# rsjahnige/CRYSTALS-Kyber

Measured on NVIDIA B200. Metric: ML-KEM-768 Encaps+Decaps ops/s, higher is better.
Workload: dtype u16/u64 integer

## Files before the change

### crystals-kyber_b200/csrc/mlkem_b200.cu

```cuda
#include "mlkem_kernels.cuh"

#include "../../include/mlkem_b200.h"

#include <algorithm>
#include <atomic>
#include <cstdio>
#include <cstdlib>
#include <cstring>
#include <mutex>
#include <vector>

namespace {

using namespace mlkem;

thread_local char tl_error[512] = "";
std::atomic<unsigned long long> g_launches{0};
int env_int(const char *name, int dflt) {
    const char *v = getenv(name);
    return v && *v ? atoi(v) : dflt;
}
constexpr int kSlots = 6;
constexpr int kDevSlots = 4;
constexpr int kHostSlots = 3;
// ... 41 lines not shown
}

#define LAUNCH(kernel, grid, block, smem, stream, ...)           \
    do {                                                         \
        auto kern_ = kernel;                                     \
        ProfEntry pe_;                                           \
        bool prof_on_;                                           \
        prof_begin(#kernel, (stream), pe_, prof_on_);            \
        kern_<<<(grid), (block), (smem), (stream)>>>(__VA_ARGS__); \
        prof_end((stream), pe_, prof_on_);                       \
        g_launches.fetch_add(1, std::memory_order_relaxed);      \
        CU(cudaGetLastError());                                  \
    } while (0)

inline unsigned cdiv(size_t a, size_t b) { return (unsigned)((a + b - 1) / b); }
inline unsigned warp_hash_grid(int n) { return cdiv((size_t)n, kWarpHashTPB / 32); }
inline unsigned warp_grid(size_t items, int warps_per_block) {
    size_t blocks = (items + warps_per_block - 1) / warps_per_block;
    const size_t cap = 148 * 16;
    return (unsigned)(blocks < cap ? blocks : cap);
}

#include "mlkem_tables.inl"

struct DeviceCtx {
    bool ready = false;
    cudaStream_t stream[kSlots] = {};
    void *ws[kSlots] = {};
    size_t ws_bytes[kSlots] = {};
    void *io[kSlots] = {};
    size_t io_bytes[kSlots] = {};
    cudaEvent_t ev_fork = nullptr, ev_join[kSlots] = {}, ev_slot[kSlots] = {};
    void *misc = nullptr;
    size_t misc_bytes = 0;
    int host_group = 0;
    std::mutex call_mutex;
    std::mutex misc_mutex;
};
DeviceCtx g_ctx[kMaxDevices];
std::mutex g_mutex;

struct DeviceGuard {
    int prev = -1;
    bool changed = false;
    int enter(int d) {
        if (cudaGetDevice(&prev) != cudaSuccess) prev = -1;
        if (prev == d) return 0;
        CU(cudaSetDevice(d));
        changed = true;
        return 0;
    }
    ~DeviceGuard() {
        if (changed && prev >= 0) cudaSetDevice(prev);
    }
};

int ensure_buffer(void **p, size_t *have, size_t need, cudaEvent_t last_use = nullptr) {
    if (*have >= need) return 0;
    if (*p) {
        if (last_use) CU(cudaEventSynchronize(last_use));
        CU(cudaMemset(*p, 0, *have));
        CU(cudaFree(*p));
    }
    *p = nullptr;
    *have = 0;
    size_t want = need + need / 8;
    CU(cudaMalloc(p, want));
    *have = want;
    return 0;
}

template <class KernelT>
int allow_smem(KernelT kernel, size_t bytes) {
    CU(cudaFuncSetAttribute(kernel, cudaFuncAttributeMaxDynamicSharedMemorySize, (int)bytes));
    CU(cudaFuncSetAttribute(kernel, cudaFuncAttributePreferredSharedMemoryCarveout, cudaSharedmemCarveoutMaxShared));
    return 0;
}
template <class P>
int allow_smem_matvec() {
    const size_t b = matvec_smem_bytes<P>();
    if (int rc = allow_smem(k_sample_matvec<P, kModeKeyGen>, b)) return rc;
    if (int rc = allow_smem(k_sample_matvec<P, kModeEncrypt>, b)) return rc;
    if (int rc = allow_smem(k_sample_matvec<P, kModeEncryptCompare>, b)) return rc;
    if (int rc = allow_smem(k_sample_matvec_list<P, kModeKeyGen>, b)) return rc;
    if (int rc = allow_smem(k_sample_matvec_list<P, kModeEncrypt>, b)) return rc;
    if (int rc = allow_smem(k_sample_matvec_list<P, kModeEncryptCompare>, b)) return rc;
    return 0;
}

int acquire(const mlkem_b200_opts *o, int *dev, DeviceCtx **ctx, DeviceGuard &guard) {
    int d = o ? o->device : -1;
    if (d < 0) CU(cudaGetDevice(&d));
    if (d >= kMaxDevices) {
        snprintf(tl_error, sizeof tl_error, "device ordinal %d out of range", d);
        return MLKEM_B200_ERR_ARG;
    }
    if (int rc = guard.enter(d)) return rc;
    std::lock_guard<std::mutex> lock(g_mutex);
    DeviceCtx &c = g_ctx[d];
    if (!c.ready) {
        cudaStream_t st[kSlots] = {};
        cudaEvent_t ev[2 * kSlots + 1] = {};
        auto create = [&]() -> int {
            TwiddleTables t;
            uint2 rc[24];
            build_tables(t, rc);
            CU(cudaMemcpyToSymbol(c_tw, &t, sizeof t));
            CU(cudaMemcpyToSymbol(g_tw, &t, sizeof t));
            CU(cudaMemcpyToSymbol(c_keccak_rc, rc, sizeof rc));
            uint32_t pow2[32];
            for (int k = 0; k < 32; k++) pow2[k] = 1u << k;
            CU(cudaMemcpyToSymbol(c_pow2, pow2, sizeof pow2));
            for (int s = 0; s < kSlots; s++) CU(cudaStreamCreateWithFlags(&st[s], cudaStreamNonBlocking));
            for (int e = 0; e < 2 * kSlots + 1; e++) CU(cudaEventCreateWithFlags(&ev[e], cudaEventDisableTiming));
            if (int r = allow_smem_matvec<P512>()) return r;
            if (int r = allow_smem_matvec<P768>()) return r;
            if (int r = allow_smem_matvec<P1024>()) return r;
            if (int r = allow_smem(k_sample_ntt_batch, 128 * kSlotWords * 4)) return r;
            return 0;
        };
        if (int r = create()) {
            for (auto s_ : st)
                if (s_) cudaStreamDestroy(s_);
            for (auto e_ : ev)
                if (e_) cudaEventDestroy(e_);
            return r;
        }
        for (int s = 0; s < kSlots; s++) {
            c.stream[s] = st[s];
            c.ev_join[s] = ev[s];
            c.ev_slot[s] = ev[kSlots + s];
        }
        c.ev_fork = ev[2 * kSlots];
        c.ready = true;
    }
    *dev = d;
    *ctx = &c;
    return 0;
}

struct Arena {
    uint8_t *base;
    size_t off = 0;
    explicit Arena(void *p) : base(static_cast<uint8_t *>(p)) {}
    template <class T>
    T *take(size_t count) {
        off = (off + 255) & ~size_t(255);
        T *p = reinterpret_cast<T *>(base + off);
        off += count * sizeof(T);
        return p;
    }
};

template <class P>
constexpr size_t ws_bytes_per_item() {
    size_t kg = 64 + 2 * P::K * 512 + 4 * P::K;
    size_t enc = P::K * 512 + (P::K + 1) * 128 + 32 + 4 * P::K;
    size_t dec = enc + 32 + 64 + 4;
    size_t m = kg > dec ? kg : dec;
    return m + 64;
}
constexpr size_t kWsSlack = 16 * 256;


template <class P, int MODE>
int launch_matvec(cudaStream_t st, Arena &ws, MatvecArgs a) {
    constexpr int K = P::K;
    const size_t rows = (size_t)a.n * K, smem = matvec_smem_bytes<P>();
    const unsigned blocks = cdiv(rows, 32), list_grid = std::min<unsigned>(blocks, 148 * 4);
#ifdef MLKEM_B200_EXPERIMENT
    static const int env_exp = env_int("MLKEM_B200_EXPERIMENT", 0);
    a.experiment = env_exp;
#endif
    if (a.group_limit >= 168 && rows > 32) {
        a.defer_list = ws.take<int>(rows);
        a.defer_count = ws.take<int>(1);
        CU(cudaMemsetAsync(a.defer_count, 0, sizeof(int), st));
        LAUNCH((k_sample_matvec<P, MODE>), blocks, 32 * K, smem, st, a);
#ifdef MLKEM_B200_EXPERIMENT
        if (env_exp & 16) return 0;
#endif
        LAUNCH((k_sample_matvec_list<P, MODE>), list_grid, 32 * K, smem, st, a);
    } else {
        a.defer_list = nullptr;
        a.defer_count = nullptr;
        LAUNCH((k_sample_matvec_list<P, MODE>), list_grid, 32 * K, smem, st, a);
    }
    return 0;
}

template <class P>
int enqueue_encrypt(cudaStream_t st, Arena &ws, int n, const uint8_t *ek, size_t ek_stride, KeySel keys, const uint8_t *m,
                    const uint8_t *seed, size_t seed_stride, uint8_t *c, const uint8_t *cmp, uint32_t *flags, int group_limit, bool fips,
                    const uint16_t *matrix = nullptr) {
    constexpr int K = P::K;
    uint16_t *yhat = ws.take<uint16_t>((size_t)n * K * 256);
    uint32_t *codes = ws.take<uint32_t>((size_t)n * (K + 1) * 32);
    if (!fips) {
        LAUNCH((k_noise<P::ETA1, true>), dim3(cdiv(n, kNoiseTPB), K), kNoiseTPB, 0, st, n, seed, seed_stride, 0, yhat, (size_t)K * 256,
               (uint32_t *)nullptr, (size_t)0, (uint8_t *)nullptr, (size_t)0, 0);
        LAUNCH((k_noise<P::ETA2, false>), dim3(cdiv(n, kNoiseTPB), K + 1), kNoiseTPB, 0, st, n, seed, seed_stride, K, (uint16_t *)nullptr,
               (size_t)0, codes, (size_t)(K + 1) * 32, (uint8_t *)nullptr, (size_t)0, 0);
    } else {
        LAUNCH((k_noise<P::ETA1, true, kRateSha3_256>), dim3(cdiv(n, kNoiseTPB), K), kNoiseTPB, 0, st, n, seed, seed_stride, 0, yhat,
               (size_t)K * 256, (uint32_t *)nullptr, (size_t)0, (uint8_t *)nullptr, (size_t)0, 0);
        LAUNCH((k_noise<P::ETA2, false, kRateSha3_256>), dim3(cdiv(n, kNoiseTPB), K + 1), kNoiseTPB, 0, st, n, seed, seed_stride, K,
               (uint16_t *)nullptr, (size_t)0, codes, (size_t)(K + 1) * 32, (uint8_t *)nullptr, (size_t)0, 0);
    }
    MatvecArgs a{};
    a.n = n;
    a.group_limit = group_limit;
    a.rho = ek + 384 * K;
    a.rho_stride = ek_stride;
    a.keys = keys;
    a.vec = yhat;
    a.vec_stride = (size_t)K * 256;
    a.addc = codes;
    a.addc_stride = (size_t)(K + 1) * 32;
    a.out = c;
    a.out_stride = P::C;
    a.cmp = cmp;
    a.flags = flags;
    EncVArgs v{};
    v.n = n;
    v.ek = ek;
    v.ek_stride = ek_stride;
    v.keys = keys;
    v.yhat = yhat;
    v.yhat_stride = (size_t)K * 256;
    v.addc = codes;
    v.addc_stride = (size_t)(K + 1) * 32;
    v.m = m;
    v.c = c;
    v.c_stride = P::C;
    v.cmp = cmp;
    v.flags = flags;
    const unsigned tgrid = warp_grid((size_t)n * K, kMatTableTPB / 32);
    if (cmp) {
        if (matrix) LAUNCH((k_matvec_table<P, kModeEncryptCompare>), tgrid, kMatTableTPB, 0, st, a, matrix);
        else if (int rc = launch_matvec<P, kModeEncryptCompare>(st, ws, a)) return rc;
        LAUNCH((k_encrypt_v<P, true>), warp_grid(n, kWarpTPB / 32), kWarpTPB, 0, st, v);
    } else {
        if (matrix) LAUNCH((k_matvec_table<P, kModeEncrypt>), tgrid, kMatTableTPB, 0, st, a, matrix);
        else if (int rc = launch_matvec<P, kModeEncrypt>(st, ws, a)) return rc;
        LAUNCH((k_encrypt_v<P, false>), warp_grid(n, kWarpTPB / 32), kWarpTPB, 0, st, v);
    }
    return 0;
}

template <class P>
int enqueue_keygen(cudaStream_t st, Arena &ws, int n, const uint8_t *d, const uint8_t *z, uint8_t *ek, uint8_t *dk, int group_limit, bool fips) {
    constexpr int K = P::K;
    const bool full = z != nullptr;
    const size_t dk_stride = full ? P::DK : P::DKPKE;
    uint8_t *rs = ws.take<uint8_t>((size_t)n * 64);
    uint16_t *se = ws.take<uint16_t>((size_t)n * 2 * K * 256);
    LAUNCH(k_keygen_G, cdiv(n, kHashTPB), kHashTPB, 0, st, n, d, (uint32_t)K, rs, ek + 384 * K, (size_t)P::EK,
           full ? dk + 768 * K : (uint8_t *)nullptr, dk_stride);
    if (!fips)
        LAUNCH((k_noise<P::ETA1, true>), dim3(cdiv(n, kNoiseTPB), 2 * K), kNoiseTPB, 0, st, n, rs + 32, (size_t)64, 0, se, (size_t)2 * K * 256,
               (uint32_t *)nullptr, (size_t)0, dk, dk_stride, K);
    else
        LAUNCH((k_noise<P::ETA1, true, kRateSha3_256>), dim3(cdiv(n, kNoiseTPB), 2 * K), kNoiseTPB, 0, st, n, rs + 32, (size_t)64, 0, se,
               (size_t)2 * K * 256, (uint32_t *)nullptr, (size_t)0, dk, dk_stride, K);
    MatvecArgs a{};
    a.n = n;
    a.group_limit = group_limit;
    a.rho = rs;
    a.rho_stride = 64;
    a.vec = se;
    a.vec_stride = (size_t)2 * K * 256;
    a.add16 = se + K * 256;
    a.add16_stride = (size_t)2 * K * 256;
    a.out = ek;
    a.out_stride = P::EK;
    a.out2 = full ? dk + 384 * K : nullptr;
    a.out2_stride = dk_stride;
    if (int rc = launch_matvec<P, kModeKeyGen>(st, ws, a)) return rc;
    if (full && n <= warp_hash_max()) LAUNCH((k_keygen_H_warp<P>), warp_hash_grid(n), kWarpHashTPB, 0, st, n, ek, z, dk);
    else if (full) LAUNCH((k_keygen_H<P>), cdiv(n, kHashTPB), kHashTPB, 0, st, n, ek, z, dk);
    return 0;
}

template <class P>
int enqueue_encaps(cudaStream_t st, Arena &ws, int n, const uint8_t *ek, const uint8_t *m, uint8_t *c, uint8_t *Kout, int group_limit, bool fips) {
    uint8_t *r = ws.take<uint8_t>((size_t)n * 32);
    if (n <= warp_hash_max()) LAUNCH((k_encaps_HG_warp<P>), warp_hash_grid(n), kWarpHashTPB, 0, st, n, ek, m, Kout, r);
    else LAUNCH((k_encaps_HG<P>), cdiv(n, kHashTPB), kHashTPB, 0, st, n, ek, m, Kout, r);
    return enqueue_encrypt<P>(st, ws, n, ek, P::EK, KeySel{}, m, r, 32, c, nullptr, nullptr, group_limit, fips);
}

template <class P>
int enqueue_encaps_keyed(cudaStream_t st, Arena &ws, int n, const uint8_t *ek, size_t ek_stride, const uint8_t *hek, KeySel keys,
                         const uint8_t *m, uint8_t *c, uint8_t *Kout, int group_limit, bool fips, const uint16_t *matrix) {
    uint8_t *r = ws.take<uint8_t>((size_t)n * 32);
    LAUNCH(k_encaps_G_keyed, cdiv(n, kHashTPB), kHashTPB, 0, st, n, hek, keys, m, Kout, r);
    return enqueue_encrypt<P>(st, ws, n, ek, ek_stride, keys, m, r, 32, c, nullptr, nullptr, group_limit, fips, matrix);
}

template <class P>
int enqueue_decaps(cudaStream_t st, Arena &ws, int n, const uint8_t *dk, KeySel keys, const uint8_t *c, uint8_t *Kout, int group_limit, bool fips,
                   const uint16_t *matrix = nullptr) {
    constexpr int K = P::K;
    uint8_t *mp = ws.take<uint8_t>((size_t)n * 32);
    uint8_t *Kr = ws.take<uint8_t>((size_t)n * 64);
    uint32_t *flags = ws.take<uint32_t>((size_t)n);
    CU(cudaMemsetAsync(flags, 0, (size_t)n * 4, st));
    LAUNCH((k_decrypt<P>), warp_grid(n, kWarpTPB / 32), kWarpTPB, 0, st, n, dk, (size_t)P::DK, keys, c, mp);
    LAUNCH((k_decaps_G<P>), cdiv(n, kHashTPB), kHashTPB, 0, st, n, mp, dk, keys, Kr);
    if (int rc = enqueue_encrypt<P>(st, ws, n, dk + 384 * K, P::DK, keys, mp, Kr + 32, 64, nullptr, c, flags, group_limit, fips, matrix)) return rc;
    if (n <= warp_hash_max()) {
        if (!fips) LAUNCH((k_decaps_J_select_warp<P>), warp_hash_grid(n), kWarpHashTPB, 0, st, n, dk, keys, c, Kr, flags, Kout);
        else LAUNCH((k_decaps_J_select_warp<P, kRateSha3_256>), warp_hash_grid(n), kWarpHashTPB, 0, st, n, dk, keys, c, Kr, flags, Kout);
        return 0;
    }
    if (!fips) LAUNCH((k_decaps_J_select<P>), cdiv(n, kHashTPB), kHashTPB, 0, st, n, dk, keys, c, Kr, flags, Kout);
    else LAUNCH((k_decaps_J_select<P, kRateSha3_256>), cdiv(n, kHashTPB), kHashTPB, 0, st, n, dk, keys, c, Kr, flags, Kout);
    return 0;
}

struct Buf {
    const void *in;
    void *out;
    size_t item_bytes;
    bool cells = false;
};

int launch_narrow(cudaStream_t st, const void *cells, void *dense, size_t bytes) {
    const size_t nw = bytes / 4;
// ... 1270 lines not shown
```

### crystals-kyber_b200/csrc/mlkem_kernels.cuh

```cuda
#pragma once
#include "mlkem_device.cuh"

namespace mlkem {

template <int K_, int ETA1_, int ETA2_, int DU_, int DV_>
struct ParamSet {
    static constexpr int K = K_, ETA1 = ETA1_, ETA2 = ETA2_, DU = DU_, DV = DV_;
    static constexpr int EK = 384 * K + 32;
    static constexpr int DKPKE = 384 * K;
    static constexpr int DK = 768 * K + 96;
    static constexpr int C1ROW = 32 * DU;
    static constexpr int C2 = 32 * DV;
    static constexpr int C = C1ROW * K + C2;
};
using P512 = ParamSet<2, 3, 2, 10, 4>;
using P768 = ParamSet<3, 2, 2, 10, 4>;
using P1024 = ParamSet<4, 2, 2, 11, 5>;

struct KeySel {
    const uint32_t *index;
    uint32_t base, nkeys;
};
__device__ __forceinline__ size_t key_row(const KeySel &k, int item) {
    if (k.index) return min(__ldg(k.index + item), k.nkeys - 1u);
// ... 329 lines not shown
#pragma unroll
    for (int m = 0; m < 4; m++) {
        uint32_t x = (t >> (6 * m)) & 7u, y = (t >> (6 * m + 3)) & 7u;
        out |= (x + 3u - y) << (4 * m);
    }
    return out;
}
__device__ __forceinline__ void cbd3_words(uint32_t w0, uint32_t w1, uint32_t w2, uint32_t &o0, uint32_t &o1) {
    uint32_t c0 = w0 & 0xFFFFFFu, c1 = (w0 >> 24) | ((w1 & 0xFFFFu) << 8), c2 = (w1 >> 16) | ((w2 & 0xFFu) << 16), c3 = w2 >> 8;
    o0 = cbd3_chunk(c0) | (cbd3_chunk(c1) << 16);
    o1 = cbd3_chunk(c2) | (cbd3_chunk(c3) << 16);
}

template <int ETA, int RATE, typename PUT>
__device__ __forceinline__ void prf_cbd_codes(const Lane seed[4], uint32_t nonce, PUT put) {
    Lane a[25];
    keccak_zero(a);
#pragma unroll
    for (int w = 0; w < 4; w++) a[w] = seed[w];
    a[4].lo = nonce | (kSfxXof << 8);
    a[RATE - 1].hi ^= 0x80000000u;
    keccak_f1600(a);
    if (ETA == 2) {
#pragma unroll
        for (int l = 0; l < 16; l++) {
            put(2 * l, cbd2_word(a[l].lo));
            put(2 * l + 1, cbd2_word(a[l].hi));
        }
    } else {
        constexpr int W1 = 2 * RATE;
        constexpr int G1 = W1 / 3;
        uint32_t o0, o1;
#pragma unroll
        for (int g = 0; g < G1; g++) {
            const int w = 3 * g;
            uint32_t w0 = (w & 1) ? a[w >> 1].hi : a[w >> 1].lo, w1 = ((w + 1) & 1) ? a[(w + 1) >> 1].hi : a[(w + 1) >> 1].lo,
                     w2 = ((w + 2) & 1) ? a[(w + 2) >> 1].hi : a[(w + 2) >> 1].lo;
            cbd3_words(w0, w1, w2, o0, o1);
            put(2 * g, o0);
            put(2 * g + 1, o1);
        }
        constexpr int LEFT = W1 - 3 * G1;
        uint32_t carry = 0;
        if (LEFT) carry = ((W1 - 1) & 1) ? a[(W1 - 1) >> 1].hi : a[(W1 - 1) >> 1].lo;
        keccak_f1600(a);
        int next = 0;
        if (LEFT) {
            cbd3_words(carry, a[0].lo, a[0].hi, o0, o1);
            put(2 * G1, o0);
            put(2 * G1 + 1, o1);
            next = 2;
        }
#pragma unroll
        for (int g = G1 + (LEFT ? 1 : 0); g < 16; g++) {
            const int w = next + 3 * (g - G1 - (LEFT ? 1 : 0));
            uint32_t w0 = (w & 1) ? a[w >> 1].hi : a[w >> 1].lo, w1 = ((w + 1) & 1) ? a[(w + 1) >> 1].hi : a[(w + 1) >> 1].lo,
                     w2 = ((w + 2) & 1) ? a[(w + 2) >> 1].hi : a[(w + 2) >> 1].lo;
            cbd3_words(w0, w1, w2, o0, o1);
            put(2 * g, o0);
            put(2 * g + 1, o1);
        }
    }
}

__device__ __forceinline__ void store_layoutC_global(const uint32_t x[8], int lane, uint16_t *dst) {
    reinterpret_cast<uint4 *>(dst)[lane] = pack_pairs(x);
}
__device__ __forceinline__ void load_layoutC_global(uint32_t x[8], int lane, const uint16_t *src) {
    unpack_pairs(__ldg(reinterpret_cast<const uint4 *>(src) + lane), x);
}

template <int ETA, bool NTT_OUT, int RATE = kRateShake128>
__global__ void __launch_bounds__(kNoiseTPB) k_noise(int n, const uint8_t *__restrict__ seeds, size_t seed_stride, int nonce0,
                                                     uint16_t *__restrict__ out16, size_t out16_stride,
                                                     uint32_t *__restrict__ outc, size_t outc_stride,
                                                     uint8_t *__restrict__ enc12, size_t enc12_stride, int enc12_polys) {
    __shared__ uint32_t s_codes[NTT_OUT ? kNoiseTPB * 33 : 1];
    __shared__ __align__(16) uint16_t s_scratch[NTT_OUT ? (kNoiseTPB / 32) * kScratchU16 : 2];
    const int p = blockIdx.y;
    const int item = blockIdx.x * kNoiseTPB + threadIdx.x;
    Lane seed[4];
#pragma unroll
    for (int w = 0; w < 4; w++) seed[w] = item < n ? load_lane(seeds + seed_stride * item + 8 * w) : Lane{0u, 0u};
    if (NTT_OUT) {
        uint32_t *mine = s_codes + 33 * threadIdx.x;
        prf_cbd_codes<ETA, RATE>(seed, (uint32_t)(nonce0 + p), [&](int w, uint32_t v) { mine[w] = v; });
        __syncwarp();
        const int lane = threadIdx.x & 31, warp = threadIdx.x >> 5;
        uint16_t *scratch = s_scratch + warp * kScratchU16;
        LaneTwiddles tw;
        load_lane_twiddles<kFmaPipe>(tw, lane);
        const uint32_t pw = nibble_weight(lane & 7);
        for (int t = 0; t < 32; t++) {
            int it = blockIdx.x * kNoiseTPB + warp * 32 + t;
            if (it >= n) break;
            const uint32_t *codes = s_codes + 33 * (warp * 32 + t) + (lane >> 3);
            uint32_t x[8];
#pragma unroll
            for (int r = 0; r < 8; r++) x[r] = nibble_fma(codes[4 * r], pw) + (kQ - 3);
            ntt_warp<kFmaPipe>(x, scratch, lane, tw);
            store_layoutC_global(x, lane, out16 + out16_stride * it + 256 * p);
            if (p < enc12_polys) {
                uint32_t *row = reinterpret_cast<uint32_t *>(enc12 + enc12_stride * it + 384 * p) + 3 * lane;
                row[0] = x[0] | (x[1] << 12) | (x[2] << 24);
                row[1] = (x[2] >> 8) | (x[3] << 4) | (x[4] << 16) | (x[5] << 28);
                row[2] = (x[5] >> 4) | (x[6] << 8) | (x[7] << 20);
            }
        }
    } else {
        if (item >= n) return;
        uint32_t buf[32];
        prf_cbd_codes<ETA, RATE>(seed, (uint32_t)(nonce0 + p), [&](int w, uint32_t v) { buf[w] = v; });
        uint4 *dst = reinterpret_cast<uint4 *>(outc + outc_stride * item + 32 * p);
#pragma unroll
        for (int v = 0; v < 8; v++) dst[v] = make_uint4(buf[4 * v], buf[4 * v + 1], buf[4 * v + 2], buf[4 * v + 3]);
    }
}

template <bool CHECKED>
__device__ __forceinline__ void parse_block(const Lane a[25], uint32_t &addr, uint32_t end_addr) {
#pragma unroll
    for (int ch = 0; ch < 7; ch++) {
        const uint32_t w[7] = {a[3 * ch].lo, a[3 * ch].hi, a[3 * ch + 1].lo, a[3 * ch + 1].hi, a[3 * ch + 2].lo, a[3 * ch + 2].hi, 0u};
#pragma unroll
        for (int m = 0; m < 16; m++) {
            const int bit = 12 * m, wi = bit >> 5, sh = bit & 31;
            uint32_t t;
            if (sh == 20) t = w[wi];
            else if (sh < 20) t = w[wi] * (1u << (20 - sh));
            else t = __funnelshift_r(w[wi], w[wi + 1], sh - 20);
            bool ok = t < (kQ << 20);
            if (CHECKED) ok = ok && (addr < end_addr);
            uint32_t d;
            asm("mul.hi.u32 %0, %1, 4096;" : "=r"(d) : "r"(t));
            if (ok) {
                asm volatile("st.shared.u16 [%0], %1;" ::"r"(addr), "h"((uint16_t)d) : "memory");
                addr += 2;
            }
        }
    }
}

__device__ __forceinline__ void mask_groups(Lane a[25], int usable) {
    const int cut = 24 * max(usable, 0);
#pragma unroll
    for (int k = 0; k < 42; k++) {
        const int lo = 32 * k;
        uint32_t m = cut <= lo ? 0xFFFFFFFFu : (cut >= lo + 32 ? 0u : (0xFFFFFFFFu << (cut - lo)));
        if (k & 1) a[k >> 1].hi |= m;
        else a[k >> 1].lo |= m;
    }
}

__device__ __forceinline__ void sample_ntt_thread(const Lane rho[4], uint32_t &b32, uint32_t &b33, uint16_t *slot, bool active,
                                                  int group_limit) {
    Lane a[25];
    const uint32_t base = (uint32_t)__cvta_generic_to_shared(slot), end_addr = base + 2 * kN;
    uint32_t addr = active ? base : end_addr;
    int groups_left = 0;
    bool need_init = true;
    while (__any_sync(kFullMask, addr < end_addr)) {
        if (need_init) {
            keccak_zero(a);
#pragma unroll
            for (int w = 0; w < 4; w++) a[w] = rho[w];
            a[4].lo = (b32 & 0xFFu) | ((b33 & 0xFFu) << 8) | (kSfxXof << 16);
            a[kRateShake128 - 1].hi ^= 0x80000000u;
            groups_left = group_limit;
            need_init = false;
        }
        keccak_f1600(a);
        const bool running = addr < end_addr;
        if (__any_sync(kFullMask, running && groups_left < 56)) {
            if (running && groups_left < 56) mask_groups(a, groups_left);
        }
        if (__all_sync(kFullMask, addr + 2 * 112 <= end_addr)) parse_block<false>(a, addr, end_addr);
        else parse_block<true>(a, addr, end_addr);
        groups_left -= 56;
        if (groups_left <= 0 && addr < end_addr) {
            b32 = (b32 + 1) & 0xFFu;
            b33 = (b33 + 1) & 0xFFu;
            addr = base;
            need_init = true;
        }
    }
}

#ifdef MLKEM_B200_EXPERIMENT
#define MLKEM_CHECK_SLOT_STORE(st, lim) \
    if ((st) + 512 < end_addr || (st) > (lim)) __trap();
#else
#define MLKEM_CHECK_SLOT_STORE(st, lim)
#endif
template <bool CHECKED>
__device__ __forceinline__ void parse_chunk3(const uint32_t w[7], uint32_t &addr, uint32_t end_addr) {
#ifndef MLKEM_B200_PARSE_ALU_ADDR
    const uint32_t one = c_pow2[0], two = c_pow2[1];
#endif
#pragma unroll
    for (int m = 0; m < 16; m++) {
        const int bit = 12 * m, wi = bit >> 5, sh = bit & 31;
        uint32_t t;
        if (sh == 20) t = w[wi];
        else if (sh < 20) t = shl_fma(w[wi], 20 - sh);
        else t = __funnelshift_r(w[wi], w[wi + 1], sh - 20);
        const bool ok = t < (kQ << 20);
        MLKEM_CHECK_SLOT_STORE(addr, CHECKED ? end_addr : end_addr - 2)
        asm volatile("st.shared.u16 [%0], %1;" ::"r"(addr), "h"((uint16_t)(t >> 20)) : "memory");
#ifndef MLKEM_B200_PARSE_ALU_ADDR
        if (CHECKED)
            asm volatile("{.reg .pred p; setp.lt.u32 p, %1, %2; setp.lt.and.u32 p, %0, %3, p; @p mad.lo.u32 %0, %4, %5, %0;}"
                         : "+r"(addr) : "r"(t), "r"(kQ << 20), "r"(end_addr), "r"(one), "r"(two));
        else
            asm volatile("{.reg .pred p; setp.lt.u32 p, %1, %2; @p mad.lo.u32 %0, %3, %4, %0;}" : "+r"(addr) : "r"(t), "r"(kQ << 20), "r"(one), "r"(two));
        (void)ok;
#else
        if (CHECKED) {
            if (ok && addr < end_addr) addr += 2;
        } else {
            if (ok) addr += 2;
        }
#endif
    }
}
template <bool CHECKED>
__device__ __forceinline__ void parse_block3(const Lane a[25], uint32_t &addr, uint32_t end_addr) {
#pragma unroll
    for (int ch = 0; ch < 7; ch++) {
        const uint32_t w[7] = {a[3 * ch].lo, a[3 * ch].hi, a[3 * ch + 1].lo, a[3 * ch + 1].hi, a[3 * ch + 2].lo, a[3 * ch + 2].hi, 0u};
        parse_chunk3<CHECKED>(w, addr, end_addr);
    }
}
__device__ __forceinline__ bool sample_ntt_three_blocks(const Lane rho[4], uint32_t b32, uint32_t b33, uint16_t *slot, int experiment = 0) {
    Lane a[25];
    const uint32_t base = (uint32_t)__cvta_generic_to_shared(slot), end_addr = base + 2 * kN;
    uint32_t addr = base;
    keccak_zero(a);
#pragma unroll
    for (int w = 0; w < 4; w++) a[w] = rho[w];
    a[4].lo = (b32 & 0xFFu) | ((b33 & 0xFFu) << 8) | (kSfxXof << 16);
    a[kRateShake128 - 1].hi ^= 0x80000000u;
#pragma unroll 1
    for (int blk = 0; blk < 3; blk++) {
        keccak_f1600(a);
#ifdef MLKEM_B200_EXPERIMENT
        if (experiment & 2) {
            addr += a[0].lo & 2;
            continue;
        }
#endif
        if (blk < 2) parse_block3<false>(a, addr, end_addr);
        else parse_block3<true>(a, addr, end_addr);
    }
    return addr >= end_addr;
}

enum MatvecMode { kModeKeyGen = 0, kModeEncrypt = 1, kModeEncryptCompare = 2 };

struct MatvecArgs {
    int n;
    int group_limit;
    const uint8_t *rho;
    size_t rho_stride;
    KeySel keys;
    const uint16_t *vec;
    size_t vec_stride;
    const uint16_t *add16;
    size_t add16_stride;
    const uint32_t *addc;
    size_t addc_stride;
    uint8_t *out;
    size_t out_stride;
    uint8_t *out2;
    size_t out2_stride;
    const uint8_t *cmp;
    uint32_t *flags;
    int *defer_list;
    int *defer_count;
#ifdef MLKEM_B200_EXPERIMENT
    int experiment;
#endif
};

constexpr int kMatvecWarpBytes = 512 + 384;
template <class P>
__host__ __device__ constexpr size_t matvec_slots_bytes() {
    return ((size_t)32 * P::K * kSlotWords * 4 + 15) & ~(size_t)15;
}
template <class P>
constexpr size_t matvec_smem_bytes() {
    return matvec_slots_bytes<P>() + (size_t)P::K * kMatvecWarpBytes + 32 * 4 + 32 * P::K;
}

struct MatvecLaneConsts {
    uint2 gam[4];
    LaneTwiddles tw;
    uint32_t pw;
};
template <int MODE>
__device__ __forceinline__ void matvec_load_consts(MatvecLaneConsts &c, int lane) {
#pragma unroll
    for (int r = 0; r < 4; r++) c.gam[r] = lane_gamma(lane + 32 * r);
    if (MODE != kModeKeyGen) load_lane_twiddles_inv<kFmaPipe>(c.tw, lane);
    c.pw = nibble_weight(lane & 7);
}
template <class P>
struct MatvecOperands {
    static constexpr int kCmpWords = (8 * P::DU + 31) / 32;
    uint32_t v[8 * P::K], cw[8], cmp[kCmpWords], ev[4];
};
template <class P, int MODE>
__device__ __forceinline__ void matvec_prefetch(MatvecOperands<P> &o, const MatvecArgs &g, int gg, int lane) {
    constexpr int K = P::K;
    if (gg < 0) return;
    const int item = gg / K, row = gg - item * K;
    const uint16_t *vec = g.vec + g.vec_stride * item;
#pragma unroll
    for (int j = 0; j < K; j++)
#pragma unroll
        for (int r = 0; r < 4; r++) {
            int t = lane + 32 * r;
            o.v[8 * j + 2 * r] = __ldg(vec + 256 * j + 2 * t);
            o.v[8 * j + 2 * r + 1] = __ldg(vec + 256 * j + 2 * t + 1);
        }
    if (MODE == kModeEncryptCompare) {
        const uint32_t *cw = reinterpret_cast<const uint32_t *>(g.cmp + g.out_stride * item + (size_t)P::C1ROW * row);
#pragma unroll
        for (int i = 0; i < MatvecOperands<P>::kCmpWords; i++) o.cmp[i] = (lane + 32 * i < 8 * P::DU) ? __ldg(cw + lane + 32 * i) : 0u;
    }
    if (MODE != kModeKeyGen) {
        const uint32_t *codes = g.addc + g.addc_stride * item + 32 * row + (lane >> 3);
#pragma unroll
        for (int r = 0; r < 8; r++) o.cw[r] = __ldg(codes + 4 * r);
    } else {
        const uint32_t *ev = reinterpret_cast<const uint32_t *>(g.add16 + g.add16_stride * item + 256 * row);
#pragma unroll
        for (int r = 0; r < 4; r++) o.ev[r] = __ldg(ev + lane + 32 * r);
    }
}

template <class P, int MODE>
__device__ __forceinline__ void matvec_row_tail(const MatvecArgs &g, int item, int row, uint32_t acc[8], const uint32_t cw8[8],
                                                const uint32_t *cmpw, const uint32_t ev4[4], uint16_t *scratch, uint8_t *stage, int lane,
                                                const LaneTwiddles &tw, uint32_t pw) {
    constexpr int kCmpWords = MatvecOperands<P>::kCmpWords;
    int nwords;
    if (MODE == kModeKeyGen) {
#pragma unroll
        for (int r = 0; r < 4; r++) {
            int t = lane + 32 * r;
            uint32_t e = ev4[r];
            uint32_t c0 = csubq(canon32(acc[2 * r]) + (e & 0xFFFFu)), c1 = csubq(canon32(acc[2 * r + 1]) + (e >> 16));
            uint32_t v = c0 | (c1 << 12);
            stage[3 * t] = (uint8_t)v;
            stage[3 * t + 1] = (uint8_t)(v >> 8);
            stage[3 * t + 2] = (uint8_t)(v >> 16);
        }
        nwords = 96;
    } else {
        uint32_t *sw = reinterpret_cast<uint32_t *>(scratch);
#pragma unroll
        for (int r = 0; r < 4; r++) {
            int t = lane + 32 * r;
            sw[sidx(2 * t) >> 1] = barrett32(acc[2 * r]) + barrett32(acc[2 * r + 1]) * 65536u;
        }
        __syncwarp();
        uint32_t x[8];
        load_scratch_C(x, scratch, lane);
        __syncwarp();
        intt_warp<kFmaPipe, false>(x, scratch, lane, tw);
#pragma unroll
        for (int r = 0; r < 8; r++) {
            uint32_t y = x[r] + nibble_fma(cw8[r], pw) + (kQ - 3);
            x[r] = compress_canon<P::DU>(canon_fma(y));
        }
        store_scratch_A(x, scratch, lane);
        __syncwarp();
        load_scratch_C(x, scratch, lane);
        pack8<P::DU>(x, stage + P::DU * lane);
        nwords = 8 * P::DU;
    }
    __syncwarp();
    const uint32_t *stw = reinterpret_cast<const uint32_t *>(stage);
    const size_t row_off = (MODE == kModeKeyGen ? 384 : P::C1ROW) * (size_t)row;
    if (MODE == kModeEncryptCompare) {
        uint32_t d = 0;
#pragma unroll
        for (int i = 0; i < kCmpWords; i++)
            if (lane + 32 * i < nwords) d |= stw[lane + 32 * i] ^ cmpw[i];
        d = __any_sync(kFullMask, d != 0) ? 1u : 0u;
        if (lane == 0) atomicOr(g.flags + item, d);
    } else {
        uint32_t *ow = reinterpret_cast<uint32_t *>(g.out + g.out_stride * item + row_off);
        for (int w = lane; w < nwords; w += 32) ow[w] = stw[w];
        if (MODE == kModeKeyGen && g.out2) {
            uint32_t *ow2 = reinterpret_cast<uint32_t *>(g.out2 + g.out2_stride * item + row_off);
            for (int w = lane; w < nwords; w += 32) ow2[w] = stw[w];
        }
    }
    __syncwarp();
}

template <class P, int MODE>
__device__ __forceinline__ void matvec_finish_rows(const MatvecArgs &g, uint32_t *s_slots, const int *s_gg, int lane, int warp,
                                                   const MatvecLaneConsts &lc, MatvecOperands<P> &nx) {
    constexpr int K = P::K;
    uint8_t *warp_area = reinterpret_cast<uint8_t *>(s_slots) + matvec_slots_bytes<P>() + warp * kMatvecWarpBytes;
    uint16_t *scratch = reinterpret_cast<uint16_t *>(warp_area);
    uint8_t *stage = warp_area + 512;
    const uint2 *gam = lc.gam;
    const LaneTwiddles &tw = lc.tw;
    const uint32_t pw = lc.pw;

    constexpr int kCmpWords = MatvecOperands<P>::kCmpWords;
#pragma unroll 1
    for (int grp = warp; grp < 32; grp += K) {
        const int gg = s_gg[grp];
        uint32_t v[8 * K], cw8[8], cmpw[kCmpWords], ev4[4];
#pragma unroll
        for (int i = 0; i < 8 * K; i++) v[i] = nx.v[i];
#pragma unroll
        for (int i = 0; i < 8; i++) cw8[i] = nx.cw[i];
#pragma unroll
        for (int i = 0; i < kCmpWords; i++) cmpw[i] = nx.cmp[i];
#pragma unroll
        for (int i = 0; i < 4; i++) ev4[i] = nx.ev[i];
        matvec_prefetch<P, MODE>(nx, g, grp + K < 32 ? s_gg[grp + K] : -1, lane);
        if (gg < 0) continue;
        const int item = gg / K, row = gg - item * K;
        const uint32_t slot0 = (uint32_t)__cvta_generic_to_shared(s_slots + kSlotWords * (grp * K));
        uint32_t acc[8];
#pragma unroll
        for (int r = 0; r < 8; r++) acc[r] = 0;
#pragma unroll
        for (int j = 0; j < K; j++) {
#pragma unroll
            for (int r = 0; r < 4; r++) {
                uint16_t a0, a1;
                const uint32_t ad = slot0 + 4 * (kSlotWords * j + lane + 32 * r);
                asm volatile("ld.shared.u16 %0, [%1];" : "=h"(a0) : "r"(ad));
                asm volatile("ld.shared.u16 %0, [%1+2];" : "=h"(a1) : "r"(ad));
                basemul_acc(acc[2 * r], acc[2 * r + 1], a0, a1, v[8 * j + 2 * r], v[8 * j + 2 * r + 1], gam[r]);
            }
        }
        matvec_row_tail<P, MODE>(g, item, row, acc, cw8, cmpw, ev4, scratch, stage, lane, tw, pw);
    }
}

template <class P>
__device__ __forceinline__ int *matvec_gg(uint32_t *s_slots) {
    return reinterpret_cast<int *>(reinterpret_cast<uint8_t *>(s_slots) + matvec_slots_bytes<P>() + P::K * kMatvecWarpBytes);
}

template <class P, int MODE>
__global__ void __launch_bounds__(32 * P::K) k_sample_matvec(MatvecArgs g) {
    constexpr int K = P::K;
    extern __shared__ __align__(16) uint32_t s_slots[];
    const int tid = threadIdx.x, lane = tid & 31, warp = tid >> 5;
    int *s_gg = matvec_gg<P>(s_slots);
    uint8_t *s_inc = reinterpret_cast<uint8_t *>(s_gg + 32);
    {
        const int grp = tid / K, col = tid - grp * K;
        const int gg = blockIdx.x * 32 + grp;
        const int item = gg / K, row = gg - item * K;
        const bool active = item < g.n;
        Lane rho[4];
#pragma unroll
        for (int w = 0; w < 4; w++) rho[w] = active ? load_lane(g.rho + g.rho_stride * key_row(g.keys, item) + 8 * w) : Lane{0u, 0u};
        const uint32_t b32 = MODE == kModeKeyGen ? col : row, b33 = MODE == kModeKeyGen ? row : col;
#ifdef MLKEM_B200_EXPERIMENT
        const bool complete = (g.experiment & 8) ? true
                                                 : sample_ntt_three_blocks(rho, b32, b33, reinterpret_cast<uint16_t *>(s_slots + kSlotWords * tid), g.experiment);
#else
        const bool complete = sample_ntt_three_blocks(rho, b32, b33, reinterpret_cast<uint16_t *>(s_slots + kSlotWords * tid));
#endif
        s_inc[tid] = active && !complete;
    }
    MatvecLaneConsts lc;
    matvec_load_consts<MODE>(lc, lane);
    MatvecOperands<P> nx;
    {
        const int gg = blockIdx.x * 32 + warp;
        matvec_prefetch<P, MODE>(nx, g, gg / K < g.n ? gg : -1, lane);
    }
    __syncthreads();
    {
        const int grp = warp + K * lane;
        if (grp < 32) {
            const int gg = blockIdx.x * 32 + grp;
            bool deferred = false;
#pragma unroll
            for (int j = 0; j < K; j++) deferred |= s_inc[grp * K + j] != 0;
            const bool active = gg / K < g.n;
            s_gg[grp] = (active && !deferred) ? gg : -1;
            if (active && deferred) g.defer_list[atomicAdd(g.defer_count, 1)] = gg;
        }
        __syncwarp();
    }
#ifdef MLKEM_B200_EXPERIMENT
    if (g.experiment & 1) return;
    if (g.experiment & 4) {
        matvec_finish_rows<P, MODE>(g, s_slots, s_gg, lane, warp, lc, nx);
        matvec_prefetch<P, MODE>(nx, g, s_gg[warp], lane);
    }
#endif
    matvec_finish_rows<P, MODE>(g, s_slots, s_gg, lane, warp, lc, nx);
}

template <class P, int MODE>
__global__ void __launch_bounds__(32 * P::K) k_sample_matvec_list(MatvecArgs g) {
    constexpr int K = P::K;
    extern __shared__ __align__(16) uint32_t s_slots[];
    const int tid = threadIdx.x, lane = tid & 31, warp = tid >> 5;
    int *s_gg = matvec_gg<P>(s_slots);
    MatvecLaneConsts lc;
    matvec_load_consts<MODE>(lc, lane);
    const int count = g.defer_list ? *g.defer_count : g.n * K;
    for (int base = blockIdx.x * 32; base < count; base += gridDim.x * 32) {
        {
            const int grp = tid / K, col = tid - grp * K;
            const int e = base + grp;
            const int gg = e < count ? (g.defer_list ? g.defer_list[e] : e) : -1;
            const bool active = gg >= 0;
            const int item = active ? gg / K : 0, row = gg - item * K;
            if (col == 0) s_gg[grp] = gg;
            Lane rho[4];
#pragma unroll
            for (int w = 0; w < 4; w++) rho[w] = active ? load_lane(g.rho + g.rho_stride * key_row(g.keys, item) + 8 * w) : Lane{0u, 0u};
            uint32_t b32 = MODE == kModeKeyGen ? col : row, b33 = MODE == kModeKeyGen ? row : col;
            sample_ntt_thread(rho, b32, b33, reinterpret_cast<uint16_t *>(s_slots + kSlotWords * tid), active, g.group_limit);
        }
        __syncthreads();
        MatvecOperands<P> nx;
        matvec_prefetch<P, MODE>(nx, g, s_gg[warp], lane);
        matvec_finish_rows<P, MODE>(g, s_slots, s_gg, lane, warp, lc, nx);
        __syncthreads();
    }
}


template <class P>
__global__ void __launch_bounds__(256) k_matrix_seeds(int n, const uint8_t *__restrict__ ek, size_t ek_stride, uint8_t *__restrict__ seeds) {
    constexpr int K = P::K;
    const int e = blockIdx.x * blockDim.x + threadIdx.x;
    if (e >= n * K * K) return;
    const int key = e / (K * K), rc = e - key * K * K, row = rc / K, col = rc - row * K;
    const uint8_t *rho = ek + ek_stride * key + 384 * K;
    uint8_t *out = seeds + 34 * (size_t)e;
    for (int b = 0; b < 32; b++) out[b] = rho[b];
    out[32] = (uint8_t)row;
    out[33] = (uint8_t)col;
}

__global__ void __launch_bounds__(256) k_scatter_rows(int n, int row_words, const uint8_t *__restrict__ src, size_t src_stride, KeySel slots,
                                                      uint8_t *__restrict__ dst, size_t dst_stride) {
    const size_t total = (size_t)n * row_words;
    for (size_t t = (size_t)blockIdx.x * blockDim.x + threadIdx.x; t < total; t += (size_t)gridDim.x * blockDim.x) {
        const int i = (int)(t / row_words), w = (int)(t - (size_t)i * row_words);
        const uint4 v = reinterpret_cast<const uint4 *>(src + src_stride * i)[w];
        reinterpret_cast<uint4 *>(dst + dst_stride * key_row(slots, i))[w] = v;
    }
}

__global__ void __launch_bounds__(kHashTPB) k_expand_seed(int n, const uint8_t *__restrict__ seed, unsigned long long first, uint32_t tag,
                                                          uint8_t *__restrict__ out0, uint8_t *__restrict__ out1) {
    const int j = blockIdx.x * blockDim.x + threadIdx.x;
    if (j >= n) return;
    const unsigned long long idx = first + (unsigned long long)j;
    Lane a[25];
    sponge_absorb_words<kRateSha3_256>(a, 6, kSfxXof, [&](int w) {
        if (w < 4) return load_lane(seed + 8 * w);
        return w == 4 ? Lane{(uint32_t)idx, (uint32_t)(idx >> 32)} : Lane{tag, 0u};
    });
#pragma unroll
    for (int w = 0; w < 4; w++) store_lane(out0 + 32 * (size_t)j + 8 * w, a[w]);
    if (out1) {
#pragma unroll
        for (int w = 0; w < 4; w++) store_lane(out1 + 32 * (size_t)j + 8 * w, a[4 + w]);
    }
}

#ifndef MLKEM_B200_MATTABLE_PREFETCH
#define MLKEM_B200_MATTABLE_PREFETCH 1
#endif
#ifndef MLKEM_B200_MATTABLE_BLOCKS
#define MLKEM_B200_MATTABLE_BLOCKS 1
#endif
template <class P, int MODE>
__global__ void __launch_bounds__(kMatTableTPB, MLKEM_B200_MATTABLE_BLOCKS) k_matvec_table(MatvecArgs g, const uint16_t *__restrict__ table) {
    static_assert(MODE != kModeKeyGen, "the table is kept in Encrypt order");
    constexpr int K = P::K, NW = kMatTableTPB / 32;
    __shared__ __align__(16) uint8_t s_warp[NW * kMatvecWarpBytes];
    const int lane = threadIdx.x & 31, warp = threadIdx.x >> 5;
    uint16_t *scratch = reinterpret_cast<uint16_t *>(s_warp + warp * kMatvecWarpBytes);
    uint8_t *stage = s_warp + warp * kMatvecWarpBytes + 512;
    MatvecLaneConsts lc;
    matvec_load_consts<MODE>(lc, lane);
    const int rows = g.n * K, stride = gridDim.x * NW;
    int gg = blockIdx.x * NW + warp;
    MatvecOperands<P> nx;
    if (MLKEM_B200_MATTABLE_PREFETCH) matvec_prefetch<P, MODE>(nx, g, gg < rows ? gg : -1, lane);
    constexpr int kCmpWords = MatvecOperands<P>::kCmpWords;
#pragma unroll 1
    for (; gg < rows; gg += stride) {
        if (!MLKEM_B200_MATTABLE_PREFETCH) matvec_prefetch<P, MODE>(nx, g, gg, lane);
        const int item = gg / K, row = gg - item * K;
        const uint32_t *arow = reinterpret_cast<const uint32_t *>(table + ((size_t)key_row(g.keys, item) * K + row) * K * 256);
        uint32_t aw[4 * K];
#pragma unroll
        for (int j = 0; j < K; j++)
#pragma unroll
            for (int r = 0; r < 4; r++) aw[4 * j + r] = __ldg(arow + 128 * j + lane + 32 * r);
        uint32_t v[8 * K], cw8[8], cmpw[kCmpWords], ev4[4];
#pragma unroll
        for (int i = 0; i < 8 * K; i++) v[i] = nx.v[i];
#pragma unroll
        for (int i = 0; i < 8; i++) cw8[i] = nx.cw[i];
#pragma unroll
        for (int i = 0; i < kCmpWords; i++) cmpw[i] = nx.cmp[i];
#pragma unroll
        for (int i = 0; i < 4; i++) ev4[i] = 0;
        if (MLKEM_B200_MATTABLE_PREFETCH) matvec_prefetch<P, MODE>(nx, g, gg + stride < rows ? gg + stride : -1, lane);
        uint32_t acc[8];
#pragma unroll
        for (int r = 0; r < 8; r++) acc[r] = 0;
#pragma unroll
        for (int j = 0; j < K; j++)
#pragma unroll
            for (int r = 0; r < 4; r++)
                basemul_acc(acc[2 * r], acc[2 * r + 1], aw[4 * j + r] & 0xFFFFu, aw[4 * j + r] >> 16, v[8 * j + 2 * r], v[8 * j + 2 * r + 1], lc.gam[r]);
        matvec_row_tail<P, MODE>(g, item, row, acc, cw8, cmpw, ev4, scratch, stage, lane, lc.tw, lc.pw);
    }
}

constexpr int kWarpTPB = 128;
#ifndef MLKEM_B200_PRIM_PIPE
#define MLKEM_B200_PRIM_PIPE false
#endif
constexpr bool kPrimPipe = MLKEM_B200_PRIM_PIPE;

struct EncVArgs {
    int n;
    const uint8_t *ek;
    size_t ek_stride;
    KeySel keys;
    const uint16_t *yhat;
    size_t yhat_stride;
    const uint32_t *addc;
    size_t addc_stride;
    const uint8_t *m;
    uint8_t *c;
    size_t c_stride;
    const uint8_t *cmp;
    uint32_t *flags;
};

__device__ __forceinline__ uint32_t smem_u32(const void *p) { return (uint32_t)__cvta_generic_to_shared(p); }
__device__ __forceinline__ void mbar_init(uint64_t *bar, int count) {
    asm volatile("mbarrier.init.shared::cta.b64 [%0], %1;" ::"r"(smem_u32(bar)), "r"(count) : "memory");
}
__device__ __forceinline__ void mbar_fence_init() { asm volatile("fence.mbarrier_init.release.cluster;" ::: "memory"); }
__device__ __forceinline__ void mbar_expect_tx(uint64_t *bar, uint32_t bytes) {
    asm volatile("mbarrier.arrive.expect_tx.shared::cta.b64 _, [%0], %1;" ::"r"(smem_u32(bar)), "r"(bytes) : "memory");
}
__device__ __forceinline__ void mbar_wait(uint64_t *bar, uint32_t parity) {
    asm volatile(
        "{\n"
        ".reg .pred p;\n"
        "WAIT_%=:\n"
        "mbarrier.try_wait.parity.shared::cta.b64 p, [%0], %1;\n"
        "@p bra DONE_%=;\n"
        "bra WAIT_%=;\n"
        "DONE_%=:\n"
        "}\n" ::"r"(smem_u32(bar)),
        "r"(parity)
        : "memory");
}
__device__ __forceinline__ void bulk_g2s(void *smem_dst, const void *gmem_src, uint32_t bytes, uint64_t *bar) {
    asm volatile("cp.async.bulk.shared::cluster.global.mbarrier::complete_tx::bytes [%0], [%1], %2, [%3];" ::"r"(smem_u32(smem_dst)),
                 "l"(gmem_src), "r"(bytes), "r"(smem_u32(bar))
                 : "memory");
}

// ... 448 lines not shown
```

Measured before the change: 33.73 million.

## Resume deferred matrix sampling from saved Keccak state instead of restarting

```diff
diff --git a/crystals-kyber_b200/csrc/mlkem_b200.cu b/crystals-kyber_b200/csrc/mlkem_b200.cu
--- a/crystals-kyber_b200/csrc/mlkem_b200.cu
+++ b/crystals-kyber_b200/csrc/mlkem_b200.cu
@@ -217,10 +217,12 @@
     }
 };
 
+constexpr size_t kResumeRowsPer = 16;
 template <class P>
 constexpr size_t ws_bytes_per_item() {
-    size_t kg = 64 + 2 * P::K * 512 + 4 * P::K;
-    size_t enc = P::K * 512 + (P::K + 1) * 128 + 32 + 4 * P::K;
+    constexpr size_t resume = (size_t)P::K * resume_record_words<P>() * 4 / kResumeRowsPer;
+    size_t kg = 64 + 2 * P::K * 512 + 4 * P::K + resume;
+    size_t enc = P::K * 512 + (P::K + 1) * 128 + 32 + 4 * P::K + resume;
     size_t dec = enc + 32 + 64 + 4;
     size_t m = kg > dec ? kg : dec;
     return m + 64;
@@ -240,6 +242,8 @@
     if (a.group_limit >= 168 && rows > 32) {
         a.defer_list = ws.take<int>(rows);
         a.defer_count = ws.take<int>(1);
+        a.resume_cap = (int)(rows / kResumeRowsPer);
+        a.resume = ws.take<uint32_t>((size_t)a.resume_cap * resume_record_words<P>());
         CU(cudaMemsetAsync(a.defer_count, 0, sizeof(int), st));
         LAUNCH((k_sample_matvec<P, MODE>), blocks, 32 * K, smem, st, a);
 #ifdef MLKEM_B200_EXPERIMENT
diff --git a/crystals-kyber_b200/csrc/mlkem_kernels.cuh b/crystals-kyber_b200/csrc/mlkem_kernels.cuh
--- a/crystals-kyber_b200/csrc/mlkem_kernels.cuh
+++ b/crystals-kyber_b200/csrc/mlkem_kernels.cuh
@@ -505,13 +505,19 @@
     }
 }
 
-__device__ __forceinline__ void sample_ntt_thread(const Lane rho[4], uint32_t &b32, uint32_t &b33, uint16_t *slot, bool active,
-                                                  int group_limit) {
-    Lane a[25];
-    const uint32_t base = (uint32_t)__cvta_generic_to_shared(slot), end_addr = base + 2 * kN;
-    uint32_t addr = active ? base : end_addr;
-    int groups_left = 0;
-    bool need_init = true;
+__device__ __forceinline__ void sample_ntt_give_up(int groups_left, uint32_t &b32, uint32_t &b33, uint32_t base, uint32_t end_addr,
+                                                   uint32_t &addr, bool &need_init) {
+    if (groups_left <= 0 && addr < end_addr) {
+        b32 = (b32 + 1) & 0xFFu;
+        b33 = (b33 + 1) & 0xFFu;
+        addr = base;
+        need_init = true;
+    }
+}
+
+__device__ __forceinline__ void sample_ntt_continue(Lane a[25], const Lane rho[4], uint32_t &b32, uint32_t &b33, uint32_t base,
+                                                    uint32_t addr, int groups_left, bool need_init, int group_limit) {
+    const uint32_t end_addr = base + 2 * kN;
     while (__any_sync(kFullMask, addr < end_addr)) {
         if (need_init) {
             keccak_zero(a);
@@ -530,13 +536,15 @@
         if (__all_sync(kFullMask, addr + 2 * 112 <= end_addr)) parse_block<false>(a, addr, end_addr);
         else parse_block<true>(a, addr, end_addr);
         groups_left -= 56;
-        if (groups_left <= 0 && addr < end_addr) {
-            b32 = (b32 + 1) & 0xFFu;
-            b33 = (b33 + 1) & 0xFFu;
-            addr = base;
-            need_init = true;
-        }
-    }
+        sample_ntt_give_up(groups_left, b32, b33, base, end_addr, addr, need_init);
+    }
+}
+
+__device__ __forceinline__ void sample_ntt_thread(const Lane rho[4], uint32_t &b32, uint32_t &b33, uint16_t *slot, bool active,
+                                                  int group_limit) {
+    Lane a[25];
+    const uint32_t base = (uint32_t)__cvta_generic_to_shared(slot);
+    sample_ntt_continue(a, rho, b32, b33, base, active ? base : base + 2 * kN, 0, true, group_limit);
 }
 
 #ifdef MLKEM_B200_EXPERIMENT
@@ -584,8 +592,8 @@
         parse_chunk3<CHECKED>(w, addr, end_addr);
     }
 }
-__device__ __forceinline__ bool sample_ntt_three_blocks(const Lane rho[4], uint32_t b32, uint32_t b33, uint16_t *slot, int experiment = 0) {
-    Lane a[25];
+__device__ __forceinline__ bool sample_ntt_three_blocks(Lane a[25], uint32_t &count, const Lane rho[4], uint32_t b32, uint32_t b33,
+                                                        uint16_t *slot, int experiment = 0) {
     const uint32_t base = (uint32_t)__cvta_generic_to_shared(slot), end_addr = base + 2 * kN;
     uint32_t addr = base;
     keccak_zero(a);
@@ -605,6 +613,7 @@
         if (blk < 2) parse_block3<false>(a, addr, end_addr);
         else parse_block3<true>(a, addr, end_addr);
     }
+    count = (addr - base) >> 1;
     return addr >= end_addr;
 }
 
@@ -630,11 +639,22 @@
     uint32_t *flags;
     int *defer_list;
     int *defer_count;
+    uint32_t *resume;
+    int resume_cap;
 #ifdef MLKEM_B200_EXPERIMENT
     int experiment;
 #endif
 };
 
+constexpr int kResumePool = 3;
+constexpr int kResumeStateWords = 52;
+constexpr int kResumeUnsaved = 0x7FFF;
+constexpr unsigned kDeferResume = 0x80000000u;
+template <class P>
+__host__ __device__ constexpr int resume_record_words() {
+    return P::K * (128 + kResumeStateWords);
+}
+
 constexpr int kMatvecWarpBytes = 512 + 384;
 template <class P>
 __host__ __device__ constexpr size_t matvec_slots_bytes() {
@@ -642,7 +662,7 @@
 }
 template <class P>
 constexpr size_t matvec_smem_bytes() {
-    return matvec_slots_bytes<P>() + (size_t)P::K * kMatvecWarpBytes + 32 * 4 + 32 * P::K;
+    return matvec_slots_bytes<P>() + (size_t)P::K * kMatvecWarpBytes + 32 * 4 + 32 * 4 * P::K + (size_t)P::K * kResumePool * kResumeStateWords * 4;
 }
 
 struct MatvecLaneConsts {
@@ -811,7 +831,8 @@
     extern __shared__ __align__(16) uint32_t s_slots[];
     const int tid = threadIdx.x, lane = tid & 31, warp = tid >> 5;
     int *s_gg = matvec_gg<P>(s_slots);
-    uint8_t *s_inc = reinterpret_cast<uint8_t *>(s_gg + 32);
+    int *s_inc = s_gg + 32;
+    uint32_t *s_pool = reinterpret_cast<uint32_t *>(s_inc + 32 * K);
     {
         const int grp = tid / K, col = tid - grp * K;
         const int gg = blockIdx.x * 32 + grp;
@@ -821,13 +842,29 @@
 #pragma unroll
         for (int w = 0; w < 4; w++) rho[w] = active ? load_lane(g.rho + g.rho_stride * key_row(g.keys, item) + 8 * w) : Lane{0u, 0u};
         const uint32_t b32 = MODE == kModeKeyGen ? col : row, b33 = MODE == kModeKeyGen ? row : col;
+        Lane a[25];
+        uint32_t count;
 #ifdef MLKEM_B200_EXPERIMENT
         const bool complete = (g.experiment & 8) ? true
-                                                 : sample_ntt_three_blocks(rho, b32, b33, reinterpret_cast<uint16_t *>(s_slots + kSlotWords * tid), g.experiment);
+                                                 : sample_ntt_three_blocks(a, count, rho, b32, b33, reinterpret_cast<uint16_t *>(s_slots + kSlotWords * tid), g.experiment);
 #else
-        const bool complete = sample_ntt_three_blocks(rho, b32, b33, reinterpret_cast<uint16_t *>(s_slots + kSlotWords * tid));
+        const bool complete = sample_ntt_three_blocks(a, count, rho, b32, b33, reinterpret_cast<uint16_t *>(s_slots + kSlotWords * tid));
 #endif
-        s_inc[tid] = active && !complete;
+        const bool incomplete = active && !complete;
+        const unsigned inc = __ballot_sync(kFullMask, incomplete);
+        int saved = -1;
+        if (incomplete) {
+            const int rank = __popc(inc & ((1u << lane) - 1u));
+            saved = kResumeUnsaved;
+            if (rank < kResumePool) {
+                saved = warp * kResumePool + rank;
+                uint2 *st = reinterpret_cast<uint2 *>(s_pool + kResumeStateWords * saved);
+#pragma unroll
+                for (int i = 0; i < 25; i++) st[i] = make_uint2(a[i].lo, a[i].hi);
+                s_pool[kResumeStateWords * saved + 50] = count;
+            }
+        }
+        s_inc[tid] = saved;
     }
     MatvecLaneConsts lc;
     matvec_load_consts<MODE>(lc, lane);
@@ -839,14 +876,40 @@
     __syncthreads();
     {
         const int grp = warp + K * lane;
+        int rec = -1;
         if (grp < 32) {
             const int gg = blockIdx.x * 32 + grp;
-            bool deferred = false;
-#pragma unroll
-            for (int j = 0; j < K; j++) deferred |= s_inc[grp * K + j] != 0;
+            bool deferred = false, saved = true;
+#pragma unroll
+            for (int j = 0; j < K; j++) {
+                const int s = s_inc[grp * K + j];
+                deferred |= s >= 0;
+                saved &= s != kResumeUnsaved;
+            }
             const bool active = gg / K < g.n;
             s_gg[grp] = (active && !deferred) ? gg : -1;
-            if (active && deferred) g.defer_list[atomicAdd(g.defer_count, 1)] = gg;
+            if (active && deferred) {
+                const int e = atomicAdd(g.defer_count, 1);
+                const bool resume = saved && e < g.resume_cap;
+                g.defer_list[e] = resume ? (int)((unsigned)gg | kDeferResume) : gg;
+                if (resume) rec = e;
+            }
+        }
+        for (unsigned todo = __ballot_sync(kFullMask, rec >= 0); todo; todo &= todo - 1) {
+            const int src = __ffs(todo) - 1, rg = warp + K * src;
+            uint32_t *dst = g.resume + (size_t)__shfl_sync(kFullMask, rec, src) * resume_record_words<P>();
+#pragma unroll
+            for (int j = 0; j < K; j++) {
+#pragma unroll
+                for (int r = 0; r < 4; r++) dst[128 * j + lane + 32 * r] = s_slots[kSlotWords * (rg * K + j) + lane + 32 * r];
+                const int s = s_inc[rg * K + j];
+                uint32_t *st = dst + 128 * K + kResumeStateWords * j;
+                if (s >= 0) {
+                    for (int w = lane; w <= 50; w += 32) st[w] = s_pool[kResumeStateWords * s + w];
+                } else if (lane == 0) {
+                    st[50] = kN;
+                }
+            }
         }
         __syncwarp();
     }
@@ -860,8 +923,12 @@
     matvec_finish_rows<P, MODE>(g, s_slots, s_gg, lane, warp, lc, nx);
 }
 
+template <class P>
+constexpr int matvec_list_min_blocks() {
+    return P::K == 2 ? 6 : (P::K == 3 ? 4 : 1);
+}
 template <class P, int MODE>
-__global__ void __launch_bounds__(32 * P::K) k_sample_matvec_list(MatvecArgs g) {
+__global__ void __launch_bounds__(32 * P::K, matvec_list_min_blocks<P>()) k_sample_matvec_list(MatvecArgs g) {
     constexpr int K = P::K;
     extern __shared__ __align__(16) uint32_t s_slots[];
     const int tid = threadIdx.x, lane = tid & 31, warp = tid >> 5;
@@ -869,11 +936,19 @@
     MatvecLaneConsts lc;
     matvec_load_consts<MODE>(lc, lane);
     const int count = g.defer_list ? *g.defer_count : g.n * K;
-    for (int base = blockIdx.x * 32; base < count; base += gridDim.x * 32) {
+    const int passes = max((count + (int)gridDim.x * 32 - 1) / ((int)gridDim.x * 32), 1);
+    const int per = g.defer_list ? (count + (int)gridDim.x * passes - 1) / ((int)gridDim.x * passes) : 32;
+    for (int base = blockIdx.x * per; base < count; base += gridDim.x * per) {
         {
             const int grp = tid / K, col = tid - grp * K;
             const int e = base + grp;
-            const int gg = e < count ? (g.defer_list ? g.defer_list[e] : e) : -1;
+            int gg = -1;
+            bool resume = false;
+            if (grp < per && e < count) {
+                const int entry = g.defer_list ? g.defer_list[e] : e;
+                gg = (int)((unsigned)entry & ~kDeferResume);
+                resume = gg != entry;
+            }
             const bool active = gg >= 0;
             const int item = active ? gg / K : 0, row = gg - item * K;
             if (col == 0) s_gg[grp] = gg;
@@ -881,7 +956,38 @@
 #pragma unroll
             for (int w = 0; w < 4; w++) rho[w] = active ? load_lane(g.rho + g.rho_stride * key_row(g.keys, item) + 8 * w) : Lane{0u, 0u};
             uint32_t b32 = MODE == kModeKeyGen ? col : row, b33 = MODE == kModeKeyGen ? row : col;
-            sample_ntt_thread(rho, b32, b33, reinterpret_cast<uint16_t *>(s_slots + kSlotWords * tid), active, g.group_limit);
+            uint32_t *slot = s_slots + kSlotWords * tid;
+            const uint32_t sbase = (uint32_t)__cvta_generic_to_shared(slot), end_addr = sbase + 2 * kN;
+            Lane a[25];
+            uint32_t addr = active ? sbase : end_addr;
+            int groups_left = 0;
+            bool need_init = true;
+            if (resume) {
+                const uint32_t *rec = g.resume + (size_t)e * resume_record_words<P>();
+                const uint4 *src = reinterpret_cast<const uint4 *>(rec + 128 * col);
+#pragma unroll 4
+                for (int v = 0; v < 32; v++) {
+                    const uint4 x = __ldg(src + v);
+                    slot[4 * v] = x.x;
+                    slot[4 * v + 1] = x.y;
+                    slot[4 * v + 2] = x.z;
+                    slot[4 * v + 3] = x.w;
+                }
+                const uint32_t *st = rec + 128 * K + kResumeStateWords * col;
+                const uint32_t have = min(__ldg(st + 50), (uint32_t)kN);
+                addr = sbase + 2 * have;
+                if (have < kN) {
+#pragma unroll
+                    for (int i = 0; i < 25; i++) {
+                        const uint2 v = __ldg(reinterpret_cast<const uint2 *>(st) + i);
+                        a[i] = Lane{v.x, v.y};
+                    }
+                    need_init = false;
+                    groups_left = g.group_limit - 3 * 56;
+                    sample_ntt_give_up(groups_left, b32, b33, sbase, end_addr, addr, need_init);
+                }
+            }
+            sample_ntt_continue(a, rho, b32, b33, sbase, addr, groups_left, need_init, g.group_limit);
         }
         __syncthreads();
         MatvecOperands<P> nx;
```

Result: no change. 33.82 million (median of 6 runs) (+0.3%).
